# toprakdeviren/gpu-bpe

Hardware: AMD Instinct MI355X
Metric: BPE merges/sec + tokenize GB/s, 1 GiB UTF-8 @ 32K vocab, 1/2/4/8 MI355X (higher is better)
Workload: dtype u16; 1 GPU; headline: 32K-vocab BPE train on 1,073,741,824 B English-like UTF-8 (seed 2, 0.5% 3-byte punctuation), heuristic word boundaries, reference compaction; step = one complete training run (trainer creation + all 32,512 merges) on the HBM-resident corpus; train_bytes=1073741824, target_vocab=32768, parallelism=single

## Files before the change

gpu-bpe_amd/csrc/common.h:

```cpp
#pragma once

#include <hip/hip_runtime.h>
#include <cstdint>
#include <cstdio>
#include <cstdlib>
#include <cstring>
#include <map>
#include <mutex>
#include <string>
#include <type_traits>
#include <unordered_map>
#include <utility>
#include <vector>

#include "../../include/gpubpe.h"

struct GbpePool {
    std::multimap<uint64_t, void*> idle;
    std::unordered_map<void*, uint64_t> busy;
    uint64_t idle_bytes = 0, hits = 0, misses = 0;
};

struct GbpeGrowBuf {
    void* p = nullptr;
// ... 68 lines not shown
        if (p && cap >= n) return hipSuccess;
        GbpeArray nb;
        hipError_t e = nb.reserve(c, n, esz);
        if (e == hipSuccess && p && keep) e = hipMemcpyAsync(nb.p, p, keep * esz, hipMemcpyDeviceToDevice, s);
        if (e == hipSuccess) e = hipStreamSynchronize(s);
        if (e == hipSuccess) *this = std::move(nb);
        return e;
    }
};

int gbpe_set_error(gbpe_ctx* ctx, int code, const char* fmt, ...);

#define GBPE_HIP(ctx, call)                                                              \
    do {                                                                                 \
        hipError_t _e = (call);                                                          \
        if (_e != hipSuccess)                                                            \
            return gbpe_set_error((ctx), _e == hipErrorOutOfMemory ? GBPE_E_OOM           \
                                                                   : GBPE_E_DEVICE,      \
                                  "%s failed: %s (%s:%d)", #call, hipGetErrorString(_e), \
                                  __FILE__, __LINE__);                                   \
    } while (0)

#define GBPE_LAUNCH_CHECK(ctx) GBPE_HIP(ctx, hipGetLastError())

__device__ __forceinline__ uint32_t gbpe_fmix32(uint32_t x) {
    x = (x ^ (x >> 16)) * 0x7feb352du;
    x = (x ^ (x >> 15)) * 0x846ca68bu;
    return x ^ (x >> 16);
}

__host__ __device__ static inline uint64_t gbpe_div_up(uint64_t a, uint64_t b) { return (a + b - 1) / b; }

constexpr const char* kGbpeDebugKeys[] = {
    "lexicon", "lex_check", "rehash", "delta_mt", "zt", "rfl", "rflz", "lxwg", "lxtwo", "pair", "pseg", "prej", "poison",
    "encode_slice", "decode_slice", "dec_plain", "me_cs", "htime", "ptrace", "rtime",
};

inline long gbpe_debug_knob(const char* key, long def) {
    const char* e = getenv("GBPE_DEBUG");
    if (!e) return def;
    const size_t kl = strlen(key);
    for (const char* p = e; *p;) {
        if (!strncmp(p, key, kl) && p[kl] == '=') return strtol(p + kl + 1, nullptr, 10);
        const char* c = strchr(p, ',');
        if (!c) break;
        p = c + 1;
    }
    return def;
}

inline std::string gbpe_debug_unknown() {
    const char* e = getenv("GBPE_DEBUG");
    for (const char* p = e ? e : ""; *p;) {
        const size_t el = strcspn(p, ","), kl = strcspn(p, ",=");
        bool ok = el == 0;
        for (const char* k : kGbpeDebugKeys) ok = ok || (kl < el && strlen(k) == kl && !strncmp(p, k, kl));
        if (!ok) return std::string(p, kl ? kl : el);
        p += el + (p[el] == ',');
    }
    return "";
}

int gbpe_pretok_gpt4_launch(gbpe_ctx* ctx, const uint8_t* d_bytes, uint64_t n, uint8_t* d_ws);
int gbpe_pretok_gpt4_docs_launch(gbpe_ctx* ctx, const uint8_t* d_bytes, uint64_t n, const uint8_t* d_flags, uint8_t* d_ws);
int gbpe_pretok_cl100k_launch(gbpe_ctx* ctx, const uint8_t* d_bytes, uint64_t n, const uint8_t* d_flags, uint8_t* d_ws);
constexpr uint32_t GBPE_DOC_BAD_ORDER = 1u, GBPE_DOC_BAD_FIRST = 2u, GBPE_DOC_BAD_LAST = 4u;
int gbpe_doc_flags_launch(gbpe_ctx* ctx, const uint64_t* d_doc_off, uint64_t n_docs, uint64_t n, uint8_t* d_flags,
// ... 8 lines not shown
```

gpu-bpe_amd/csrc/sparse.h:

```cpp
#pragma once

#include "train_dev.h"

namespace {

constexpr uint32_t SP_WPW_MIN = 16;
constexpr uint32_t SP_CH = 256;
constexpr uint32_t SP_INV = 0xFFFFFFFFu;
constexpr uint32_t SP_SHRINKS = 64;
constexpr uint32_t SP_SHRINKS_MAX = 1024;
constexpr uint32_t SP_SECW = 256;
constexpr uint32_t SP_DIV = 64;
constexpr uint32_t SP_LX_DIV = 16;
constexpr uint32_t SP_SHRINK_PCT = 200;
constexpr uint32_t SP_ZONE_F = 3;
constexpr uint32_t SP_SUB_ZONE = 1u << 20;
constexpr uint32_t SP_SUB_K = 16;
constexpr uint32_t SP_ZSEG_LO = 8192;
constexpr uint32_t SP_BODY_SUB = 4;
constexpr uint32_t SP_BODY_MIN = 256;

constexpr uint32_t SP_SIGW = 64;
__device__ __forceinline__ uint32_t sig_hash(uint32_t pid) { return gbpe_fmix32(pid ^ 0x9E3779B9u); }
__device__ __forceinline__ void sig_bits(uint32_t pid, uint32_t& b1, uint32_t& b2, uint32_t& b3) {
// ... 499 lines not shown
        for (int k = 1; k < ZPT; ++k) xv = k == hk ? x[k] : xv;
        s_last = ((rwm >> hk) & 1u) ? (nw | (xv & WS)) : xv;
    }
    asm volatile("s_waitcnt vmcnt(0)" ::: "memory");
    __syncthreads();
    if (t == 0) {
        constexpr unsigned long long TAG = 1ull << 32;
        __hip_atomic_store(&zg->gran[seg][0], TAG | Ks, __ATOMIC_RELAXED, __HIP_MEMORY_SCOPE_AGENT);
        __hip_atomic_store(&zg->gran[seg][1], TAG | Ts, __ATOMIC_RELAXED, __HIP_MEMORY_SCOPE_AGENT);
        __hip_atomic_store(&zg->gran[seg][2], TAG | (Ks ? (s_last | 0x80000000u) : 0u), __ATOMIC_RELAXED,
                           __HIP_MEMORY_SCOPE_AGENT);
        KT(7);
    }
    constexpr uint32_t PV = 16 / sizeof(S), PVL = sizeof(S) == 2 ? 3 : 2;
    auto swz = [](uint32_t o) -> uint32_t {
        const uint32_t c = o >> PVL;
        return ((c ^ ((c >> 3) & 7u)) << PVL) | (o & (PV - 1u));
    };
    uint32_t wsm = 0;
#pragma unroll
    for (int k = 0; k < ZPT; ++k) {
        const bool rw = (rwm >> k) & 1u;
        const uint32_t v = rw ? (nw | (x[k] & WS)) : x[k];
        wsm |= ((x[k] & WS) ? 1u : 0u) << k;
        const uint32_t o = pre + (uint32_t)__popc(keep & ((1u << k) - 1u));
        S* dst = ((keep >> k) & 1u) ? &xs[swz(o)] : &L.trash[lane];
        *dst = (S)v;
    }
    for (uint32_t r = rwm; r; r &= r - 1) {
        const int k = __ffs(r) - 1;
        zc[gi0 + k] = (S)(nw | (((wsm >> k) & 1u) ? WS : 0u));
    }
    if (wid == 0) {
        uint32_t gk = 0, gt = 0, gl = 0;
        for (uint32_t it = 0;; ++it) {
            bool ok = true;
            if ((uint32_t)lane < nz) {
                const unsigned long long x0 = __hip_atomic_load(&zg->gran[lane][0], __ATOMIC_RELAXED, __HIP_MEMORY_SCOPE_AGENT);
                const unsigned long long x1 = __hip_atomic_load(&zg->gran[lane][1], __ATOMIC_RELAXED, __HIP_MEMORY_SCOPE_AGENT);
                const unsigned long long x2 = __hip_atomic_load(&zg->gran[lane][2], __ATOMIC_RELAXED, __HIP_MEMORY_SCOPE_AGENT);
                ok = (x0 >> 32) == 1u && (x1 >> 32) == 1u && (x2 >> 32) == 1u;
                gk = (uint32_t)x0;
                gt = (uint32_t)x1;
                gl = (uint32_t)x2;
            }
            if (__all(ok)) break;
            if (it > ZSEG_SPIN) {
                if (lane == 0) atomicOr(&st->err, ERR_SPIN);
                break;
            }
            __builtin_amdgcn_s_sleep(1);
        }
        const bool in = (uint32_t)lane < nz;
        uint32_t sp = in && (uint32_t)lane < seg ? gk : 0u, sk = in ? gk : 0u, stt = in ? gt : 0u;
        sp = wave_sum_u32(sp);
        sk = wave_sum_u32(sk);
        stt = wave_sum_u32(stt);
        const unsigned long long hm = __ballot(in && (gl >> 31));
        if (lane == 0) {
            s_pre = sp;
            s_kz = sk;
            s_m = EXACT ? 0u : stt;
            s_x0 = 0u;
        }
        if (hm && lane == 63 - __clzll(hm)) s_x0 = gl & 0x7FFFFFFFu;
    }
    __syncthreads();
    if (t == 0) KT(8);
    const uint32_t P = s_pre, Kz = s_kz, m = s_m;
    for (uint32_t j = t; j < Ks; j += BT) zo[P + j] = xs[swz(j)];
    if (!EXACT && m) {
        const uint32_t w0 = mc - m, f = q0 ? q0 - 1u : 0u;
        const uint32_t lo = q0 > w0 ? q0 : w0;
        for (uint32_t q = lo + t; q < q1; q += BT) {
            const uint32_t x1 = L.wb[q - f];
            const uint32_t x0 = q == w0 ? s_x0 : (uint32_t)L.wb[q - 1u - f];
            zo[Kz + (q - w0)] = (S)x1;
            if (!(x1 & WS) && (x0 & TM) && (x1 & TM)) lds_add(lt, tb, st, ((x0 & TM) << 16) | (x1 & TM), 1u);
        }
    }
    if (t == 0) KT(9);
    lds_flush(lt, tb, st);
    if (t == 0) {
        KT(4);
        if (seg == 0) {
            zst->m = m;
            zst->valid_total = Kz + m + 1u;
        }
        const uint32_t ws = q1 > q0 ? q1 - q0 : 0u;
        atomicAdd(bytes, (uint64_t)sizeof(S) * ((uint64_t)nh + Ks + 2u * ws + (EXACT ? 0u : mc / nz)));
    }
}

struct SelShard {
    uint32_t zf = SP_ZONE_F;
    uint32_t sub = 1;
    uint32_t k2 = 0;
    uint32_t prej = 0;
// ... 1149 lines not shown
```

gpu-bpe_amd/csrc/train.hip:

```cpp


#include <chrono>
#include "trainer.h"

int trainer_create_impl(gbpe_ctx* ctx, const uint8_t* bytes, uint64_t n, const uint8_t* word_starts,
                        int input_on_device, const gbpe_train_opts* opts, uint64_t cap_extra, gbpe_trainer** out,
                        const StateInit* si) {
    if (!ctx || !out || !opts) return gbpe_set_error(ctx, GBPE_E_INVALID, "null argument");
    *out = nullptr;
    if (n == 0) return gbpe_set_error(ctx, GBPE_E_EMPTY, "No symbols to train on — corpus is empty after pre-processing");
    if (!bytes) return gbpe_set_error(ctx, GBPE_E_INVALID, "bytes is null");
    if (n >= 0xFFFFFFF0ull) return gbpe_set_error(ctx, GBPE_E_INVALID, "corpus too large for one device (%llu symbols)", (unsigned long long)n);
    const auto t_create0 = std::chrono::steady_clock::now();
    auto* t = new (std::nothrow) gbpe_trainer();
    if (!t) return gbpe_set_error(ctx, GBPE_E_OOM, "host allocation failed");
    if (const int rc = trainer_config(t, ctx, opts)) {
        delete t;
        return rc;
    }
    const uint32_t next_id = t->next_id0;
    t->bps = t->u16 ? 2 : 4;
    t->n0 = n;
    t->n = (uint32_t)n;
    hipStream_t s = ctx->stream;
// ... 205 lines not shown
            t->ht_filters += std::chrono::duration<double, std::micro>(std::chrono::steady_clock::now() - a0).count();
            ++t->ht_nfilters;
        }
    }
    if (!t->sp && t->h_st->enter_lim && t->n >= (1u << 24)) k = 1;
    if (t->sp && (uint32_t)t->n - t->h_st->B > SP_SUB_ZONE && k > SP_SUB_K) k = SP_SUB_K;
    DevState* hs = t->h_st.p;
    hs->merges_done = 0;
    hs->budget = k;
    if (t->sp) hs->sel_round = 0;
    hipLaunchKernelGGL(k_step_in, dim3(1), dim3(1), 0, s, t->st.p, t->sp ? t->zst.p : (DevState*)nullptr, k);
#ifdef GBPE_KTRACE
    if (getenv("GBPE_KTRACE_OUT")) {
        static unsigned long long* kbuf = nullptr;
        if (!kbuf) {
            const size_t nb = (size_t)(KT_MERGES / KT_EVERY) * 2 * KT_WG * KT_SLOTS * 8;
            TR_HIP(t, dev_malloc(t->ctx, &kbuf, nb));
            TR_HIP(t, hipMemsetAsync(kbuf, 0, nb, s));
            TR_HIP(t, hipMemcpyToSymbolAsync(HIP_SYMBOL(g_ktr), &kbuf, sizeof(kbuf), 0, hipMemcpyHostToDevice, s));
        }
        const uint32_t kb = (uint32_t)t->done;
        TR_HIP(t, hipMemcpyToSymbolAsync(HIP_SYMBOL(g_kt_base), &kb, 4, 0, hipMemcpyHostToDevice, s));
    }
#endif
    const uint64_t ntiles = gbpe_div_up(t->n, TILE);
    const uint32_t g_tail = (t->flags & GBPE_TRAIN_EXACT_COMPACTION) ? 0u
                            : grid_persistent(t->ctx, gbpe_div_up(t->n / 2 + 1, TPB * 16), 1);
    const uint32_t g_delta = (uint32_t)(ntiles ? ntiles : 1);
    const uint32_t g_compact = (uint32_t)ntiles + g_tail;
    uint32_t g_refresh = t->g_refresh;
    const bool timing = (t->flags & GBPE_TRAIN_TIMING) != 0;
    const bool sparse = t->sp;
    SpGrid sg{};
    if (sparse) {
        const uint32_t zn = (uint32_t)t->n - hs->B;
        const uint64_t zt = gbpe_div_up(zn, TILE);
        const uint32_t z256 = t->u16 ? zone_max<uint16_t>(256) : zone_max<uint32_t>(256);
        sg.bt = zn <= z256 ? 256 : 1024;
        body_grid(t, sg.bt, &sg.body, &sg.wpg, 0, &sg.sub);
        if (sg.bt == 1024 && t->u16 && zn <= 16384u) sg.bt = 1023;
        sg.zone1 = zn <= (t->u16 ? zone_max<uint16_t>(sg.bt) : zone_max<uint32_t>(sg.bt)) ? 1u : 0u;
        const bool p16 = t->pair_on && t->pair16_on && t->zseg.p && k >= 2 && zn > SP_ZSEG_LO && zn <= SP_PAIR16_HI;
        if (p16) {
            sg.bt = 1022;
            sg.zone1 = 1;
        } else if (t->zseg.p && zn > SP_ZSEG_LO && zn <= NSEG_MAX * 16384u) {
            sg.seg8 = zn <= NSEG_MAX * 8192u;
            sg.zone1 = (uint32_t)gbpe_div_up(zn, sg.seg8 ? 8192u : 16384u);
        }
        sg.copy = (t->flags & GBPE_TRAIN_EXACT_COMPACTION) ? 0u : grid_persistent(t->ctx, gbpe_div_up(zn / 5 + 1, TPB * 8), 1);
        sg.zdelta = (uint32_t)(zt ? zt : 1);
        sg.zcompact = (uint32_t)zt + ((t->flags & GBPE_TRAIN_EXACT_COMPACTION) ? 0u
                                      : grid_persistent(t->ctx, gbpe_div_up(zn / 2 + 1, TPB * 16), 1));
        const uint32_t extra = p16 ? ((t->flags & GBPE_TRAIN_EXACT_COMPACTION) ? 1u : 2u) : sg.zone1 ? sg.zone1 : sg.copy;
        if (sg.bt >= 1022 && extra && sg.body + extra > t->body_cap && 2 * extra <= t->body_cap)
            body_grid(t, sg.bt, &sg.body, &sg.wpg, t->body_cap - extra, &sg.sub);
        if (t->refresh_late && zn <= t->refresh_late_z) {
            const uint32_t want = std::min<uint32_t>(t->tb.nblk,
                                                     std::max<uint32_t>(t->refresh_late, (uint32_t)gbpe_div_up(t->tb.nblk, TPB)));
            if (want != t->g_refresh) {
                t->g_refresh = g_refresh = want;
                if (t->u16)
                    GBPE_LAUNCH_REFRESH(uint16_t, want, t->tb.nblk, s, t->st.p, 0u, 0, t->tb, (uint16_t*)nullptr,
                                        (const uint32_t*)nullptr, (DevState*)nullptr, (uint32_t*)nullptr, FusedSel(),
                                        t->part.p, (uint32_t*)nullptr);
                else
                    GBPE_LAUNCH_REFRESH(uint32_t, want, t->tb.nblk, s, t->st.p, 0u, 0, t->tb, (uint32_t*)nullptr,
                                        (const uint32_t*)nullptr, (DevState*)nullptr, (uint32_t*)nullptr, FusedSel(),
                                        t->part.p, (uint32_t*)nullptr);
                GBPE_LAUNCH_CHECK(t->ctx);
            }
        }
        sg.refresh = g_refresh;
        sg.pair = t->pair_on && sg.zone1 == 1 && (sg.bt == 256 || sg.bt == 1022) && t->zseg.p && k >= 2;
    }
    uint32_t nl = k;
    if (sg.pair) nl = std::min<uint32_t>(k, (uint32_t)std::ceil((double)k / (1.0 + t->pair_rate)) + 2u);
    const uint32_t paired0 = hs->paired;
    auto launch_all = [&]() -> int {
        for (uint32_t r = 0; r < nl; ++r) {
            hipEvent_t* ev = timing ? &t->evs[5 * r] : nullptr;
            int rc;
            if (sparse)
                rc = t->u16 ? launch_merge_sparse<uint16_t>(t, r, s, sg, timing, ev)
                            : launch_merge_sparse<uint32_t>(t, r, s, sg, timing, ev);
            else
                rc = t->u16 ? launch_merge<uint16_t>(t, r, s, g_delta, g_compact, g_refresh, timing, ev)
                            : launch_merge<uint32_t>(t, r, s, g_delta, g_compact, g_refresh, timing, ev);
            if (rc != GBPE_OK) return rc;
        }
        return GBPE_OK;
    };
    const auto h0 = std::chrono::steady_clock::now();
    auto h1 = h0;
    {
        int rc = launch_all();
        if (rc != GBPE_OK) return rc;
        h1 = std::chrono::steady_clock::now();
        const bool cl = sparse && t->d_clog.p;
        hipLaunchKernelGGL(k_step_out, dim3(1), dim3(1024), 0, s, t->st.p, sparse ? t->zst.p : (DevState*)nullptr, t->tb,
                           sparse ? 1 : 0, (const uint32_t*)t->d_log.p, k * 4u, (const uint32_t*)(cl ? t->d_clog.p : nullptr),
                           cl ? k * 2u : 0u, t->h_st.p, t->h_zst.p, t->h_log.p, cl ? t->h_clog.p : (uint32_t*)nullptr);
        GBPE_LAUNCH_CHECK(t->ctx);
    }
    TR_HIP(t, hipStreamSynchronize(s));
    const uint32_t done = hs->merges_done;
    {
        const uint32_t dbl = hs->paired - paired0;
        t->pair_done += dbl;
        if (sg.pair && done > dbl) t->pair_rate = (double)dbl / (double)(done - dbl);
        if (t->ptrace)
            fprintf(stderr, "[ptrace] merge %u zone %u zone1 %u bt %d pair %d launches %u done %u paired %u cand %u mc %u us %.1f\n",
                    t->done, hs->n - hs->B, sg.zone1, sg.bt, sg.pair ? 1 : 0, nl, done, dbl,
                    hs->pair_cand, done ? t->h_log.p[(done - 1) * 4 + 3] : 0u,
                    std::chrono::duration<double, std::micro>(std::chrono::steady_clock::now() - hs0).count());
    }
    if (t->htime) {
        t->ht_pre += std::chrono::duration<double, std::micro>(h0 - hs0).count();
        const double enq = std::chrono::duration<double, std::micro>(h1 - h0).count();
        const double wait = std::chrono::duration<double, std::micro>(std::chrono::steady_clock::now() - h1).count();
        t->ht_enq += enq;
        t->ht_wait += wait;
        ++t->ht_steps;
        if (sparse && (uint32_t)t->n - hs->B <= 16384u) {
            t->ht_enq_late += enq;
            t->ht_wait_late += wait;
            ++t->ht_steps_late;
            t->ht_merges_late += done;
        }
    }
#ifdef GBPE_BSPROF
    if (sparse && getenv("GBPE_BSPROF")) {
        unsigned long long h[8] = {0, 0, 0, 0, 0, 0, 0, 0};
        TR_HIP(t, hipMemcpyFromSymbol(h, HIP_SYMBOL(g_bsprof), sizeof(h), 0, hipMemcpyDeviceToHost));
        fprintf(stderr, "[bsprof] merges %u-%u waves %llu sectors %llu passes %llu | cyc/sector loads+hits %.0f deltas %.0f "
                        "writes %.0f flush %.0f | sector-phase cyc/wave %.0f\n",
                (unsigned)t->done, (unsigned)(t->done + done), h[7], h[5], h[4], h[5] ? (double)h[0] / h[5] : 0.0,
                h[5] ? (double)h[1] / h[5] : 0.0, h[5] ? (double)h[2] / h[5] : 0.0, h[5] ? (double)h[3] / h[5] : 0.0,
                h[7] ? (double)h[6] / h[7] : 0.0);
        const unsigned long long z[8] = {0, 0, 0, 0, 0, 0, 0, 0};
        TR_HIP(t, hipMemcpyToSymbol(HIP_SYMBOL(g_bsprof), z, sizeof(z), 0, hipMemcpyHostToDevice));
    }
#endif
    const uint32_t err = hs->err | (sparse ? t->h_zst->err : 0u);
    if (err) {
        return gbpe_set_error(t->ctx, GBPE_E_INTERNAL, "training invariant violated (err=0x%x: %s%s%s%s%s)", err,
                              (err & ERR_TABLE_FULL) ? "pair table full " : "",
                              (err & ERR_COUNT_MISMATCH) ? "survivor count mismatch " : "",
// ... 334 lines not shown
```

gpu-bpe_amd/csrc/train_dev.h:

```cpp
#pragma once

#include "common.h"
#include "scan.h"

#include <algorithm>
#include <chrono>
#include <type_traits>
#include <cstdarg>

namespace {

constexpr int TPB = 256;
constexpr int EPT = 32;
constexpr int TILE = TPB * EPT;
constexpr int LTAB = 2048;
constexpr int LTAB_FULL = 8192;
constexpr int LPROBE = 24;
constexpr uint32_t BLK_LOG2 = 8;
constexpr int SEL_THREADS = 1024;

template <typename S> struct Sym;
template <> struct Sym<uint16_t> { static constexpr uint32_t WS = 0x8000u, TM = 0x7FFFu; };
template <> struct Sym<uint32_t> { static constexpr uint32_t WS = 0x10000u, TM = 0xFFFFu; };

// ... 67 lines not shown
    uint32_t ndirty;
    uint32_t err;
    uint32_t valid_total;
    uint32_t budget;
    uint32_t live;
    uint64_t tail_total;
    uint32_t max_live;
    uint32_t epoch;
    uint32_t B;
    uint32_t Bp;
    uint32_t body_rm;
    uint32_t sp_abort;
    uint32_t sel_round;
    uint64_t sp_bytes;
    uint32_t zlast;
    uint32_t is_last;
    uint32_t cand;
    uint32_t hitsec;
    uint32_t mc_prev;
    uint32_t enter_lim;
    uint32_t mc2;
    uint32_t body_rm2;
    uint32_t acc2;
    uint32_t paired;
    uint32_t pair_cand;
    uint32_t pair_rej;
};
static_assert(sizeof(DevState) <= 256, "state");

__device__ __forceinline__ uint64_t win_src0(const DevState& g, uint32_t mc) {
    return (uint64_t)(uint32_t)(g.n - g.Bp) - 2ull * mc;
}

constexpr uint32_t NSEG_MAX = 64;
constexpr uint32_t ZSEG_SPIN = 1u << 22;
struct ZSegState {
    uint32_t ticket;
    uint32_t pad[15];
    unsigned long long gran[NSEG_MAX][4];
};
constexpr uint32_t ZSEG_WORDS = 16 + NSEG_MAX * 8;

#ifdef GBPE_KTRACE
constexpr uint32_t KT_MERGES = 40000, KT_EVERY = 16, KT_WG = 2048, KT_SLOTS = 12;
__constant__ unsigned long long* g_ktr;
__constant__ uint32_t g_kt_base;
__device__ __forceinline__ void kt_put(uint32_t round, uint32_t wg, int i, unsigned long long v) {
    const uint32_t m = g_kt_base + round;
    if (g_ktr && m < KT_MERGES && m % KT_EVERY == 0 && wg < 2 * KT_WG)
        g_ktr[((uint64_t)(m / KT_EVERY) * 2 * KT_WG + wg) * KT_SLOTS + i] = v;
}
#define KT(i) kt_put(round, blockIdx.x, (i), wall_clock64())
#define KTV(i, v) kt_put(round, blockIdx.x, (i), (v))
#define KTR(i) kt_put(round, KT_WG + blockIdx.x, (i), wall_clock64())
#define KTW(i) do { if ((threadIdx.x & 63) == 0 && threadIdx.x < 256) kt_put(round, KT_WG - 8u + (threadIdx.x >> 6), (i), wall_clock64()); } while (0)
#define KTC(i) do { if ((threadIdx.x & 63) == 0 && threadIdx.x < 256) kt_put(round, KT_WG - 4u + (threadIdx.x >> 6), (i), wall_clock64()); } while (0)
#else
#define KTW(i) ((void)0)
#define KTC(i) ((void)0)
#define KT(i) ((void)0)
#define KTV(i, v) ((void)0)
#define KTR(i) ((void)0)
#endif

#ifdef GBPE_BSPROF
__device__ unsigned long long g_bsprof[8];
#define BSP_ARG , unsigned long long (&bsp)[6]
#define BSP_PASS , bsp
#define BSP_CLK(v) const unsigned long long v = clock64()
#define BSP_ADD(i, x) bsp[i] += (x)
#else
#define BSP_ARG
#define BSP_PASS
#define BSP_CLK(v) ((void)0)
// ... 441 lines not shown
            if (i0 + k < n && i0 + k > 0 && !(x & Sym<S>::WS) && t0 && t1 && (t0 >> 7) == half)
                atomicAdd(&hist[((t0 & 127u) << 8) | t1], 1u);
            prev = x;
        }
    }
    __syncthreads();
    for (int i = threadIdx.x; i < 32768; i += CB_T) {
        const uint32_t c = hist[i];
        if (c) atomicAdd(&gh[(half << 15) | (uint32_t)i], c);
    }
}

__device__ void table_add(const Table& tb, DevState* st, uint32_t pid, uint32_t delta);
__global__ __launch_bounds__(256) void k_count_hist(const uint32_t* __restrict__ gh, DevState* st, Table tb) {
    const uint32_t i = blockIdx.x * 256u + threadIdx.x;
    const uint32_t c = gh[i];
    if (c) table_add(tb, st, ((i >> 8) << 16) | (i & 255u), c);
}

__device__ void select_merge(DevState* st, Table tb, uint32_t* __restrict__ log, uint32_t* __restrict__ grpsum,
                             DevState* zst, uint32_t exact);

struct FusedSel {
    uint32_t* log = nullptr;
    uint32_t* grpsum = nullptr;
    uint32_t exact = 0;
};


template <typename S, bool WIDE = false>
__global__ __launch_bounds__(TPB) void k_refresh(DevState* st, uint32_t round, int finish, Table tb, S* __restrict__ cur,
                                                 const uint32_t* __restrict__ rwlist, DevState* zst,
                                                 uint32_t* __restrict__ clog = nullptr, FusedSel fs = FusedSel(),
                                                 uint64_t* __restrict__ part = nullptr, uint32_t* __restrict__ zseg = nullptr) {
    (void)cur;
    if (zseg && blockIdx.x == 0)
        for (uint32_t i = threadIdx.x; i < ZSEG_WORDS; i += TPB)
            if (i == 0 || i >= 16) zseg[i] = 0u;
    (void)rwlist;
    if (part && finish == 2 && threadIdx.x == 0) KTR(0);
    __shared__ uint64_t s_dmask[WIDE ? TPB / 64 : 1];
    __shared__ uint64_t s_bm[WIDE ? TPB : 64], s_bm2[WIDE ? TPB : 64];
    const uint32_t per = (tb.nblk + gridDim.x - 1) / gridDim.x;
    constexpr bool wide = WIDE;
    const uint32_t b0 = blockIdx.x * per;
    uint64_t f_bm = 0ull, f_bm2 = 0ull;
    bool f_d = false;
    if (wide || threadIdx.x < 64) {
        const uint32_t blk = b0 + threadIdx.x;
        const bool in = threadIdx.x < per && blk < tb.nblk;
        if (part && in) {
            f_bm = tb.bmax[blk];
            f_bm2 = tb.bmax2[blk];
        }
        f_d = in && tb.dirty[blk];
    }
    if (finish && blockIdx.x == 0) {
        constexpr int NW = sizeof(DevState) / 4;
        __shared__ union {
            DevState d;
            uint32_t w[NW];
        } s_g, s_z;
        static_assert(64 + 2 * NW <= TPB, "state snapshot beside the flag loads");
        if (threadIdx.x >= 64 && threadIdx.x < 64 + NW)
            s_g.w[threadIdx.x - 64] = reinterpret_cast<const uint32_t*>(st)[threadIdx.x - 64];
        else if (zst && threadIdx.x >= 64 + NW && threadIdx.x < 64 + 2 * NW)
            s_z.w[threadIdx.x - 64 - NW] = reinterpret_cast<const uint32_t*>(zst)[threadIdx.x - 64 - NW];
        __syncthreads();
        const DevState& g = s_g.d;
        const DevState& z = s_z.d;
        const uint32_t r = finish >= 2 ? g.merges_done : round;
// ... 996 lines not shown
```

gpu-bpe_amd/csrc/trainer.h:

```cpp
#pragma once

#include <cmath>

#include "train_dev.h"
#include <chrono>
#include "sparse.h"




struct gbpe_trainer {
    gbpe_ctx* ctx = nullptr;
    bool u16 = true;
    uint32_t bps = 2;
    uint64_t n0 = 0, cap_syms = 0;
    uint64_t n_prev0 = 0;
    uint32_t next_id0 = 256;
    GbpeArray<void> buf[2];
    int cur = 0;
    uint64_t n = 0;
    uint32_t needed = 0, done = 0;
    bool stop = false;
    uint32_t flags = 0, batch = GBPE_BATCH_SIZE;
    GbpeArray<DevState> st;
// ... 30 lines not shown
    int zcur = 0;
    GbpeArray<DevState> zst;
    GbpeArray<DevState, true> h_zst;
    GbpeArray<uint32_t> d_u32;
    GbpeArray<uint64_t> part;
    GbpeArray<uint2> zdr_out;
    GbpeArray<uint32_t> zdr_offs, zdr_flag;
    uint32_t zdr_ntile = 0;
    GbpeArray<uint32_t> zseg;
    uint32_t table_grows = 0;
    GbpeArray<uint64_t> wg_bytes;
    uint32_t delta_mt = 2048;
    double ms_sparse = 0, ms_dense = 0;
    double ms_body = 0;
    double ms_create = 0;
    uint64_t dense_bytes = 0;
    uint32_t g_refresh = 0;
    uint64_t sp_merges = 0, sp_sectors = 0, sp_zone = 0;
    uint32_t sp_enters = 0, sp_exits = 0;
    uint32_t sp_cooldown = 0;
    GbpeArray<uint32_t> d_bhist;
    uint32_t lx_wg = 16384;
    bool lx_two = true;
    uint32_t lx_resize = 0;
    uint32_t sp_zt = 5;
    uint32_t refresh_late = 64;
    uint32_t refresh_late_z = 16384;
    bool rehash_on = true;
    uint32_t body_cap = 256;
    bool pair_on = true;
    double pair_rate = 0.5;
    uint64_t pair_done = 0;
    bool pair16_on = true;
    uint32_t pair_prej = 0;
    uint32_t ptrace = 0;
    GbpeArray<uint32_t> d_clog;
    GbpeArray<uint32_t, true> h_clog;
    FILE* trace = nullptr;
    uint32_t htime = 0;
    double ht_enq = 0, ht_wait = 0, ht_enq_late = 0, ht_wait_late = 0, ht_pre = 0, ht_post = 0, ht_out = 0;
    double ht_shrink = 0, ht_filters = 0, ht_grow = 0;
    uint64_t ht_nshrink = 0, ht_nfilters = 0;
    std::chrono::steady_clock::time_point ht_last{};
    uint64_t ht_steps = 0, ht_steps_late = 0, ht_merges_late = 0;
    bool lex = false;
    bool lex_on = true;
    bool lex_only = false;
    GbpeArray<void> lx_store;
    GbpeArray<uint32_t> lx_mul;
    uint64_t lx_len = 0;
    GbpeArray<uint32_t> lx_occ;
    uint64_t lx_nocc = 0;
    GbpeArray<uint32_t> lx_w0;
    uint32_t lx_nuid = 0;
    GbpeArray<void> lx_tmp;
    uint64_t lx_words = 0, lx_builds = 0, lx_fallbacks = 0;
};

namespace {

int tr_err(gbpe_trainer* t, int code, const char* msg) { return gbpe_set_error(t->ctx, code, "%s", msg); }

#define TR_HIP(t, call) GBPE_HIP((t)->ctx, call)

inline void* sp_body(const gbpe_trainer* t) { return t->lex ? t->lx_store.p : t->buf[t->bcur].p; }
inline uint32_t* sp_mul(const gbpe_trainer* t) { return t->lex ? t->lx_mul.p : nullptr; }
// ... 136 lines not shown
                               t->hitmask.p, t->tile_cnt.p, t->grpsum.p, g_delta, 0xFFFFFFFFu);
        if (timing) TR_HIP(t, hipEventRecord(ev[3], s));
        hipLaunchKernelGGL((k_compact<S, true>), dim3(g_compact), dim3(CTPB), 0, s, t->st.p, round, cur, oth,
                           (const uint32_t*)t->hitmask.p, (const uint32_t*)t->tile_cnt.p, (const uint32_t*)t->grpsum.p, t->tb);
    } else {
        if (mt)
            hipLaunchKernelGGL((k_delta_mt<S, false, 8>), dim3(g_mt + g_mtail), dim3(TPB), 0, s, t->st.p, round,
                               (const S*)cur, t->tb, t->hitmask.p, t->tile_cnt.p, t->grpsum.p, g_delta, g_mt, 0u, ZdrView());
        else
            hipLaunchKernelGGL((k_delta<S, false>), dim3(g_delta + g_dtail), dim3(TPB), 0, s, t->st.p, round, (const S*)cur,
                               t->tb, t->hitmask.p, t->tile_cnt.p, t->grpsum.p, g_delta, g_delta);
        if (timing) TR_HIP(t, hipEventRecord(ev[3], s));
        hipLaunchKernelGGL((k_compact<S, false>), dim3(g_compact), dim3(CTPB), 0, s, t->st.p, round, cur, oth,
                           (const uint32_t*)t->hitmask.p, (const uint32_t*)t->tile_cnt.p, (const uint32_t*)t->grpsum.p, t->tb);
    }
    if (timing) TR_HIP(t, hipEventRecord(ev[2], s));
    FusedSel fs;
    fs.log = nullptr;
    fs.grpsum = t->grpsum.p;
    fs.exact = exact ? 1u : 0u;
    GBPE_LAUNCH_REFRESH(S, g_refresh, t->tb.nblk, s, t->st.p, round, 1, t->tb, cur, (const uint32_t*)nullptr,
                        (DevState*)nullptr, (uint32_t*)nullptr, fs, (uint64_t*)nullptr, (uint32_t*)nullptr);
    if (timing) TR_HIP(t, hipEventRecord(ev[4], s));
    GBPE_LAUNCH_CHECK(t->ctx);
    return GBPE_OK;
}


struct SpGrid {
    uint32_t body, copy, zdelta, zcompact, refresh;
    uint32_t wpg = 16;
    uint32_t sub = 1;
    bool seg8 = false;
    uint32_t zone1;
    int bt;
    bool pair = false;
};

constexpr uint32_t SP_PAIR16_HI = 16384;

template <typename S>
uint32_t zone_max(int bt) {
    return bt == 1023 ? 1024u * 16u : bt == 1022 ? SP_PAIR16_HI : bt == 1024 ? ZoneDim<S, 1024>::ZMAX : ZoneDim<S, 256>::ZMAX;
}
inline void body_grid(const gbpe_trainer* t, int bt, uint32_t* nbody, uint32_t* wpg, uint32_t cap = 0,
                      uint32_t* sub = nullptr) {
    const uint32_t W = (uint32_t)gbpe_div_up(t->nsec, 32);
    const uint32_t minw = bt == 1024 ? 32u : 16u;
    uint32_t g = (uint32_t)gbpe_div_up(W, minw);
    const uint32_t gmin = std::min<uint32_t>(W, SP_BODY_MIN);
    if (g < gmin) g = gmin;
    if (g > (cap ? cap : t->body_cap)) g = cap ? cap : t->body_cap;
    if (g == 0) g = 1;
    *wpg = (uint32_t)gbpe_div_up(W, g);
    if (*wpg == 0) *wpg = 1;
    *nbody = (uint32_t)gbpe_div_up(W, *wpg);
    if (*nbody == 0) *nbody = 1;
    if (sub) {
        *sub = 1;
        const uint32_t c = cap ? cap : t->body_cap;
        while (*sub * 2 <= SP_BODY_SUB && (uint64_t)W * *sub * 2 <= c) *sub *= 2;
        if (*sub > 1) {
            *wpg = 1;
            *nbody = W * *sub;
        }
    }
}

template <typename S, bool EXACT, typename... A>
void launch_body(int bt, uint32_t grid, hipStream_t s, A... args) {
    if (bt == 1022)
        hipLaunchKernelGGL((k_body<S, EXACT, 512, 32, false, true>), dim3(grid), dim3(512), 0, s, args...);
    else if (bt == 2048)
        hipLaunchKernelGGL((k_body<S, EXACT, 1024, 16, true>), dim3(grid), dim3(1024), 0, s, args...);
    else if (bt == 2049)
        hipLaunchKernelGGL((k_body<S, EXACT, 1024, 8, true>), dim3(grid), dim3(1024), 0, s, args...);
    else if (bt == 1023 && sizeof(S) == 2)
        hipLaunchKernelGGL((k_body<S, EXACT, 1024, 16>), dim3(grid), dim3(1024), 0, s, args...);
    else if (bt >= 1023)
        hipLaunchKernelGGL((k_body<S, EXACT, 1024>), dim3(grid), dim3(1024), 0, s, args...);
    else
        hipLaunchKernelGGL((k_body<S, EXACT, 256>), dim3(grid), dim3(256), 0, s, args...);
}

template <typename S>
int launch_merge_sparse(gbpe_trainer* t, uint32_t round, hipStream_t s, const SpGrid& g, bool timing, hipEvent_t* ev) {
    S* zc = (S*)t->zbuf[t->zcur ^ (round & 1)].p;
    S* zo = (S*)t->zbuf[t->zcur ^ (round & 1) ^ 1].p;
    const bool exact = (t->flags & GBPE_TRAIN_EXACT_COMPACTION) != 0;
    if (timing) TR_HIP(t, hipEventRecord(ev[0], s));
    if (timing) TR_HIP(t, hipEventRecord(ev[1], s));
    const bool inbody = g.zone1 >= 2;
    const uint32_t z1 = g.zone1;
    const int bt = inbody ? (g.seg8 ? 2049 : 2048) : g.bt;
    SelShard sh;
    sh.sub = g.sub;
    sh.k2 = g.pair ? 1u : 0u;
    sh.prej = t->pair_prej;
    sh.churn = (g.pair && !exact && (bt == 256 || bt == 1022) && z1 == 1) ? 1u : 0u;
    const uint32_t gb = g.body + (g.zone1 ? g.zone1 : g.copy) + sh.churn;
    if ((uint64_t)g.body + 1 > t->wg_bytes.cap)
        return gbpe_set_error(t->ctx, GBPE_E_INTERNAL, "k_body grid (%u) above its byte counters (%llu)", g.body,
                              (unsigned long long)t->wg_bytes.cap);
    S* zb0 = (S*)t->zbuf[t->zcur].p;
    S* zb1 = (S*)t->zbuf[t->zcur ^ 1].p;
    if (exact)
        launch_body<S, true>(bt, gb, s, t->st.p, round, (S*)sp_body(t), t->sec.p, t->bits.p, t->W, g.wpg, t->sig.p, t->tb,
                             g.body, zb1, (S*)t->wtmp.p, t->d_clog.p ? 1u : 0u, t->zst.p, zb0, z1,
                             (const uint64_t*)t->part.p, g.refresh, t->d_log.p, t->grpsum.p, t->wg_bytes.p, t->tb, sh,
                             sp_mul(t), (ZSegState*)t->zseg.p);
    else
        launch_body<S, false>(bt, gb, s, t->st.p, round, (S*)sp_body(t), t->sec.p, t->bits.p, t->W, g.wpg, t->sig.p, t->tb,
                              g.body, zb1, (S*)t->wtmp.p, t->d_clog.p ? 1u : 0u, t->zst.p, zb0, z1,
                              (const uint64_t*)t->part.p, g.refresh, t->d_log.p, t->grpsum.p, t->wg_bytes.p, t->tb, sh,
                              sp_mul(t), (ZSegState*)t->zseg.p);
    if (timing) TR_HIP(t, hipEventRecord(ev[3], s));
    if (!g.zone1 && !exact) {
        const bool mt = t->delta_mt && g.zdelta >= t->delta_mt;
        const uint32_t g_mt = (uint32_t)gbpe_div_up(g.zdelta, 8);
        const uint32_t ntw = mt ? g_mt : g.zdelta;
        const uint32_t gch = (uint32_t)std::min<uint64_t>(ZDR_P, std::max<uint64_t>(1, gbpe_div_up(((uint32_t)t->n - t->h_st->B) / 5 + 1, 16384)));
        ZdrView zv;
        zv.out = t->zdr_out.p;
        zv.offs = t->zdr_offs.p;
        zv.flag = t->zdr_flag.p;
        zv.ntile = ntw;
        zv.tag = (uint32_t)(t->done + round + 1);
        if (ntw > t->zdr_ntile) return gbpe_set_error(t->ctx, GBPE_E_INTERNAL, "zone delta dumps too small");
        if (mt)
            hipLaunchKernelGGL((k_delta_mt<S, false, 8>), dim3(g_mt), dim3(TPB), 0, s, t->zst.p, round, (const S*)zc, t->tb,
                               t->hitmask.p, t->tile_cnt.p, t->grpsum.p, g.zdelta, g_mt, 0u, zv);
        else
            hipLaunchKernelGGL((k_delta<S, false, true>), dim3(g.zdelta), dim3(TPB), 0, s, t->zst.p, round, (const S*)zc,
                               t->tb, t->hitmask.p, t->tile_cnt.p, t->grpsum.p, g.zdelta, g.zdelta, zv);
        hipLaunchKernelGGL((k_compact<S, false, true>), dim3(g.zdelta), dim3(CTPB), 0, s, t->zst.p, round, zc, zo,
                           (const uint32_t*)t->hitmask.p, (const uint32_t*)t->tile_cnt.p, (const uint32_t*)t->grpsum.p, t->tb,
                           (const S*)t->wtmp.p, (const DevState*)t->st.p, 1u);
        hipLaunchKernelGGL(k_churn<S>, dim3(gch), dim3(CH_BT), 0, s, t->zst.p, round, zc, zo, (const uint32_t*)t->hitmask.p,
                           (const uint32_t*)t->grpsum.p, (const S*)t->wtmp.p, t->tb, zv, ntw);
        hipLaunchKernelGGL(k_zdr, dim3(ZDR_P), dim3(TPB), 0, s, zv, ntw + gch, t->tb, t->zst.p, round);
    } else if (!g.zone1) {
        const uint32_t g_mt = (uint32_t)gbpe_div_up(g.zdelta, 8);
        if (t->delta_mt && g.zdelta >= t->delta_mt)
            hipLaunchKernelGGL((k_delta_mt<S, true, 8>), dim3(g_mt), dim3(TPB), 0, s, t->zst.p, round, (const S*)zc, t->tb,
                               t->hitmask.p, t->tile_cnt.p, t->grpsum.p, g.zdelta, g_mt);
        else
            hipLaunchKernelGGL((k_delta<S, true, true>), dim3(g.zdelta), dim3(TPB), 0, s, t->zst.p, round, (const S*)zc,
                               t->tb, t->hitmask.p, t->tile_cnt.p, t->grpsum.p, g.zdelta, 0xFFFFFFFFu);
        hipLaunchKernelGGL((k_compact<S, true, true>), dim3(g.zcompact), dim3(CTPB), 0, s, t->zst.p, round, zc, zo,
                           (const uint32_t*)t->hitmask.p, (const uint32_t*)t->tile_cnt.p, (const uint32_t*)t->grpsum.p,
                           t->tb, (const S*)t->wtmp.p, (const DevState*)t->st.p);
    }
    if (timing) TR_HIP(t, hipEventRecord(ev[2], s));
    GBPE_LAUNCH_REFRESH(S, g.refresh, t->tb.nblk, s, t->st.p, round, 2, t->tb, (S*)nullptr, (const uint32_t*)nullptr,
                        t->zst.p, t->d_clog.p, FusedSel(), t->part.p, t->zseg.p);
    if (timing) TR_HIP(t, hipEventRecord(ev[4], s));
    GBPE_LAUNCH_CHECK(t->ctx);
    return GBPE_OK;
}

__global__ void k_restride(const uint32_t* __restrict__ old, uint32_t w_old, uint32_t* __restrict__ nb, uint32_t w_new,
                           uint64_t rows) {
    const uint64_t tot = rows * w_new;
    for (uint64_t i = (uint64_t)blockIdx.x * blockDim.x + threadIdx.x; i < tot; i += (uint64_t)gridDim.x * blockDim.x) {
        const uint64_t r = i / w_new, w = i % w_new;
        nb[i] = w < w_old ? old[r * w_old + w] : 0u;
    }
}

int sp_scratch(gbpe_trainer* t, uint64_t cap) {
    TR_HIP(t, t->sp_loc.reserve(t->ctx, cap));
    TR_HIP(t, t->sp_blk.reserve(t->ctx, gbpe_div_up(cap, SCAN_BLK) + 1));
    return GBPE_OK;
}

int sp_wg_bytes(gbpe_trainer* t, uint64_t W) {
    hipStream_t s = t->ctx->stream;
    const uint64_t need = std::max<uint64_t>(gbpe_div_up(W, SP_WPW_MIN), t->body_cap) + 2, had = t->wg_bytes.cap;
    if (need <= had) return GBPE_OK;
    TR_HIP(t, t->wg_bytes.reserve_keep(t->ctx, need, had, s));
    TR_HIP(t, hipMemsetAsync(t->wg_bytes.p + had, 0, (need - had) * sizeof(uint64_t), s));
    return GBPE_OK;
}

int sp_reserve(gbpe_trainer* t, uint64_t need_sec, uint64_t need_store, uint64_t need_occ) {
    hipStream_t s = t->ctx->stream;
    if (need_sec > t->sec.cap || need_sec > (uint64_t)t->W * 32 || need_sec * SP_SIGW > t->sig.cap ||
        need_sec > t->sp_loc.cap || (t->lex && need_sec > t->lx_w0.cap)) {
// ... 608 lines not shown
    uint64_t sl = t->zbuf[0].cap;
    if (Bp + sl > t->cap_syms) sl = t->cap_syms - Bp;
    TR_HIP(t, hipMemcpyAsync(body + Bp, t->zbuf[t->zcur ^ 1].p, sl * t->bps, hipMemcpyDeviceToDevice, s));
    hs->sp_abort = 0;
    TR_HIP(t, hipMemcpyAsync(&t->st->sp_abort, &hs->sp_abort, 4, hipMemcpyHostToDevice, s));
    TR_HIP(t, hipStreamSynchronize(s));
    if (btot != B) return gbpe_set_error(t->ctx, GBPE_E_INTERNAL, "sparse exit: body sectors hold %llu symbols, expected %u",
                                         (unsigned long long)btot, B);
    t->cur = t->bcur ^ 1;
    t->sp = false;
    t->lex = false;
    ++t->sp_exits;
    return GBPE_OK;
}

int trainer_config(gbpe_trainer* t, gbpe_ctx* ctx, const gbpe_train_opts* opts) {
    const std::string bad = gbpe_debug_unknown();
    if (!bad.empty()) return gbpe_set_error(ctx, GBPE_E_INVALID, "GBPE_DEBUG: unknown key '%s'", bad.c_str());
    t->ctx = ctx;
    t->flags = opts->flags;
    t->batch = opts->batch_size ? opts->batch_size : GBPE_BATCH_SIZE;
    const uint32_t vocab_size = opts->vocab_size ? opts->vocab_size : 256u;
    const uint32_t next_id = opts->next_token_id ? opts->next_token_id : 256u;
    t->next_id0 = next_id;
    t->needed = opts->target_vocab_size > vocab_size ? opts->target_vocab_size - vocab_size : 0u;
    const uint64_t max_id = (uint64_t)next_id + t->needed;
    t->u16 = max_id <= 0x8000ull;
    t->max_id = (uint32_t)(max_id < 0x10000ull ? max_id : 0x10000ull);
    t->body_cap = (uint32_t)(ctx->num_cu > 0 ? ctx->num_cu : 256);
    t->lex_on = gbpe_debug_knob("lexicon", 1) != 0;
    t->pair_on = gbpe_debug_knob("pair", 1) != 0;
    t->pair16_on = gbpe_debug_knob("pseg", 1) != 0;
    t->pair_prej = (uint32_t)std::max<long>(0, gbpe_debug_knob("prej", 0));
    t->ptrace = (uint32_t)gbpe_debug_knob("ptrace", 0);
    t->rehash_on = gbpe_debug_knob("rehash", 1) != 0;
    t->delta_mt = (uint32_t)gbpe_debug_knob("delta_mt", t->delta_mt);
    t->sp_zt = (uint32_t)gbpe_debug_knob("zt", t->sp_zt);
    t->refresh_late = (uint32_t)gbpe_debug_knob("rfl", t->refresh_late);
    t->refresh_late_z = (uint32_t)gbpe_debug_knob("rflz", t->refresh_late_z);
    t->lx_wg = (uint32_t)std::max<long>(1, gbpe_debug_knob("lxwg", t->lx_wg));
    t->lx_two = gbpe_debug_knob("lxtwo", 1) != 0;
    t->htime = (uint32_t)gbpe_debug_knob("htime", 0);
    if (t->sp_zt < SP_ZONE_F) t->sp_zt = SP_ZONE_F;
    if (const char* e = getenv("GBPE_SPARSE_TRACE")) {
        t->trace = fopen(e, "w");
        if (t->trace && (t->d_clog.reserve(ctx, (size_t)t->batch * 2) != hipSuccess ||
                         t->h_clog.reserve(ctx, (size_t)t->batch * 2) != hipSuccess))
            t->d_clog.release(), t->h_clog.release();
    }
    t->bps = t->u16 ? 2 : 4;
    return GBPE_OK;
}

int sp_exit_any(gbpe_trainer* t) { return !t->sp ? GBPE_OK : (t->u16 ? sp_exit<uint16_t>(t) : sp_exit<uint32_t>(t)); }

}

struct StateInit {
    const uint32_t* prev;
    uint64_t n_prev;
};
int trainer_create_impl(gbpe_ctx* ctx, const uint8_t* bytes, uint64_t n, const uint8_t* word_starts,
                        int input_on_device, const gbpe_train_opts* opts, uint64_t cap_extra, gbpe_trainer** out,
                        const StateInit* si = nullptr);
```

Before: 64790 merges/s.

## Extend segmented zone body to 128 segments and add 32K-segment u16 variant

Raises the segmented-zone cap from 64 to 128 segments, limited by CU count, and adds a seg32 path that uses 32768-element segments for u16 symbols. The in-kernel cross-segment scan now handles two granules per lane when there are more than 64 segments. The refresh kernel clears only as many zseg words as are in use. The aim is to keep larger zones on the single-launch segmented body path instead of falling back to the slower non-segmented path. The cost is a more complex spin-wait over more granules and heavier per-thread work in the seg32 body.

Measured after the change: 66390 merges/s (median of 6 runs). +2.5%, better.

```diff
diff --git a/gpu-bpe_amd/csrc/common.h b/gpu-bpe_amd/csrc/common.h
--- a/gpu-bpe_amd/csrc/common.h
+++ b/gpu-bpe_amd/csrc/common.h
@@ -124,7 +124,7 @@
 __host__ __device__ static inline uint64_t gbpe_div_up(uint64_t a, uint64_t b) { return (a + b - 1) / b; }
 
 constexpr const char* kGbpeDebugKeys[] = {
-    "lexicon", "lex_check", "rehash", "delta_mt", "zt", "rfl", "rflz", "lxwg", "lxtwo", "pair", "pseg", "prej", "poison",
+    "lexicon", "lex_check", "rehash", "delta_mt", "zt", "rfl", "rflz", "lxwg", "lxtwo", "pair", "pseg", "prej", "zsmax", "zs32", "poison",
     "encode_slice", "decode_slice", "dec_plain", "me_cs", "htime", "ptrace", "rtime",
 };
 
diff --git a/gpu-bpe_amd/csrc/sparse.h b/gpu-bpe_amd/csrc/sparse.h
--- a/gpu-bpe_amd/csrc/sparse.h
+++ b/gpu-bpe_amd/csrc/sparse.h
@@ -555,38 +555,66 @@
         zc[gi0 + k] = (S)(nw | (((wsm >> k) & 1u) ? WS : 0u));
     }
     if (wid == 0) {
-        uint32_t gk = 0, gt = 0, gl = 0;
-        for (uint32_t it = 0;; ++it) {
-            bool ok = true;
-            if ((uint32_t)lane < nz) {
-                const unsigned long long x0 = __hip_atomic_load(&zg->gran[lane][0], __ATOMIC_RELAXED, __HIP_MEMORY_SCOPE_AGENT);
-                const unsigned long long x1 = __hip_atomic_load(&zg->gran[lane][1], __ATOMIC_RELAXED, __HIP_MEMORY_SCOPE_AGENT);
-                const unsigned long long x2 = __hip_atomic_load(&zg->gran[lane][2], __ATOMIC_RELAXED, __HIP_MEMORY_SCOPE_AGENT);
-                ok = (x0 >> 32) == 1u && (x1 >> 32) == 1u && (x2 >> 32) == 1u;
-                gk = (uint32_t)x0;
-                gt = (uint32_t)x1;
-                gl = (uint32_t)x2;
-            }
-            if (__all(ok)) break;
-            if (it > ZSEG_SPIN) {
-                if (lane == 0) atomicOr(&st->err, ERR_SPIN);
-                break;
-            }
-            __builtin_amdgcn_s_sleep(1);
-        }
-        const bool in = (uint32_t)lane < nz;
+        const uint32_t sh = (uint32_t)lane + 64u;
+        const bool in = (uint32_t)lane < nz, inh = sh < nz;
+        const bool up = nz > 64u;
+        uint32_t gk = 0, gt = 0, gl = 0, hk = 0, ht = 0, hl = 0;
+        auto sweep = [&](auto two) {
+            constexpr bool TWO = decltype(two)::value;
+            for (uint32_t it = 0;; ++it) {
+                bool ok = true;
+                if (in) {
+                    const unsigned long long x0 = __hip_atomic_load(&zg->gran[lane][0], __ATOMIC_RELAXED, __HIP_MEMORY_SCOPE_AGENT);
+                    const unsigned long long x1 = __hip_atomic_load(&zg->gran[lane][1], __ATOMIC_RELAXED, __HIP_MEMORY_SCOPE_AGENT);
+                    const unsigned long long x2 = __hip_atomic_load(&zg->gran[lane][2], __ATOMIC_RELAXED, __HIP_MEMORY_SCOPE_AGENT);
+                    ok = (x0 >> 32) == 1u && (x1 >> 32) == 1u && (x2 >> 32) == 1u;
+                    gk = (uint32_t)x0;
+                    gt = (uint32_t)x1;
+                    gl = (uint32_t)x2;
+                    if constexpr (TWO) {
+                        if (inh) {
+                            const unsigned long long y0 = __hip_atomic_load(&zg->gran[sh][0], __ATOMIC_RELAXED, __HIP_MEMORY_SCOPE_AGENT);
+                            const unsigned long long y1 = __hip_atomic_load(&zg->gran[sh][1], __ATOMIC_RELAXED, __HIP_MEMORY_SCOPE_AGENT);
+                            const unsigned long long y2 = __hip_atomic_load(&zg->gran[sh][2], __ATOMIC_RELAXED, __HIP_MEMORY_SCOPE_AGENT);
+                            ok = ok && (y0 >> 32) == 1u && (y1 >> 32) == 1u && (y2 >> 32) == 1u;
+                            hk = (uint32_t)y0;
+                            ht = (uint32_t)y1;
+                            hl = (uint32_t)y2;
+                        }
+                    }
+                }
+                if (__all(ok)) break;
+                if (it > ZSEG_SPIN) {
+                    if (lane == 0) atomicOr(&st->err, ERR_SPIN);
+                    break;
+                }
+                __builtin_amdgcn_s_sleep(1);
+            }
+        };
+        if (up) sweep(std::true_type());
+        else sweep(std::false_type());
         uint32_t sp = in && (uint32_t)lane < seg ? gk : 0u, sk = in ? gk : 0u, stt = in ? gt : 0u;
+        if (up) {
+            sp += inh && sh < seg ? hk : 0u;
+            sk += inh ? hk : 0u;
+            stt += inh ? ht : 0u;
+        }
         sp = wave_sum_u32(sp);
         sk = wave_sum_u32(sk);
         stt = wave_sum_u32(stt);
         const unsigned long long hm = __ballot(in && (gl >> 31));
+        const unsigned long long hmh = up ? __ballot(inh && (hl >> 31)) : 0ull;
         if (lane == 0) {
             s_pre = sp;
             s_kz = sk;
             s_m = EXACT ? 0u : stt;
             s_x0 = 0u;
         }
-        if (hm && lane == 63 - __clzll(hm)) s_x0 = gl & 0x7FFFFFFFu;
+        if (hmh) {
+            if (lane == 63 - __clzll(hmh)) s_x0 = hl & 0x7FFFFFFFu;
+        } else if (hm && lane == 63 - __clzll(hm)) {
+            s_x0 = gl & 0x7FFFFFFFu;
+        }
     }
     __syncthreads();
     if (t == 0) KT(8);
diff --git a/gpu-bpe_amd/csrc/train.hip b/gpu-bpe_amd/csrc/train.hip
--- a/gpu-bpe_amd/csrc/train.hip
+++ b/gpu-bpe_amd/csrc/train.hip
@@ -261,6 +261,7 @@
     const bool timing = (t->flags & GBPE_TRAIN_TIMING) != 0;
     const bool sparse = t->sp;
     SpGrid sg{};
+    const uint32_t zn0 = sparse ? (uint32_t)t->n - hs->B : 0u;
     if (sparse) {
         const uint32_t zn = (uint32_t)t->n - hs->B;
         const uint64_t zt = gbpe_div_up(zn, TILE);
@@ -273,9 +274,13 @@
         if (p16) {
             sg.bt = 1022;
             sg.zone1 = 1;
-        } else if (t->zseg.p && zn > SP_ZSEG_LO && zn <= NSEG_MAX * 16384u) {
-            sg.seg8 = zn <= NSEG_MAX * 8192u;
+        } else if (t->zseg.p && zn > SP_ZSEG_LO && zn <= t->zseg_max * 16384u &&
+                   !(t->u16 && t->zseg32 == 2 && zn > 64u * 16384u)) {
+            sg.seg8 = zn <= std::min<uint32_t>(t->zseg_max, 64u) * 8192u;
             sg.zone1 = (uint32_t)gbpe_div_up(zn, sg.seg8 ? 8192u : 16384u);
+        } else if (t->zseg.p && t->u16 && t->zseg32 && zn > SP_ZSEG_LO && zn <= t->zseg_max * 32768u) {
+            sg.seg32 = true;
+            sg.zone1 = (uint32_t)gbpe_div_up(zn, 32768u);
         }
         sg.copy = (t->flags & GBPE_TRAIN_EXACT_COMPACTION) ? 0u : grid_persistent(t->ctx, gbpe_div_up(zn / 5 + 1, TPB * 8), 1);
         sg.zdelta = (uint32_t)(zt ? zt : 1);
@@ -339,10 +344,10 @@
         t->pair_done += dbl;
         if (sg.pair && done > dbl) t->pair_rate = (double)dbl / (double)(done - dbl);
         if (t->ptrace)
-            fprintf(stderr, "[ptrace] merge %u zone %u zone1 %u bt %d pair %d launches %u done %u paired %u cand %u mc %u us %.1f\n",
-                    t->done, hs->n - hs->B, sg.zone1, sg.bt, sg.pair ? 1 : 0, nl, done, dbl,
+            fprintf(stderr, "[ptrace] merge %u zone %u zone1 %u bt %d pair %d launches %u done %u paired %u cand %u mc %u us %.1f zone0 %u\n",
+                    t->done, hs->n - hs->B, sg.zone1, sg.seg32 ? 2050 : sg.bt, sg.pair ? 1 : 0, nl, done, dbl,
                     hs->pair_cand, done ? t->h_log.p[(done - 1) * 4 + 3] : 0u,
-                    std::chrono::duration<double, std::micro>(std::chrono::steady_clock::now() - hs0).count());
+                    std::chrono::duration<double, std::micro>(std::chrono::steady_clock::now() - hs0).count(), zn0);
     }
     if (t->htime) {
         t->ht_pre += std::chrono::duration<double, std::micro>(h0 - hs0).count();
diff --git a/gpu-bpe_amd/csrc/train_dev.h b/gpu-bpe_amd/csrc/train_dev.h
--- a/gpu-bpe_amd/csrc/train_dev.h
+++ b/gpu-bpe_amd/csrc/train_dev.h
@@ -123,14 +123,14 @@
     return (uint64_t)(uint32_t)(g.n - g.Bp) - 2ull * mc;
 }
 
-constexpr uint32_t NSEG_MAX = 64;
+constexpr uint32_t NSEG_MAX = 128;
 constexpr uint32_t ZSEG_SPIN = 1u << 22;
 struct ZSegState {
     uint32_t ticket;
     uint32_t pad[15];
     unsigned long long gran[NSEG_MAX][4];
 };
-constexpr uint32_t ZSEG_WORDS = 16 + NSEG_MAX * 8;
+__host__ __device__ constexpr uint32_t zseg_words(uint32_t nz) { return nz >= 2 ? 16u + (nz < NSEG_MAX ? nz : NSEG_MAX) * 8u : 1u; }
 
 #ifdef GBPE_KTRACE
 constexpr uint32_t KT_MERGES = 40000, KT_EVERY = 16, KT_WG = 2048, KT_SLOTS = 12;
@@ -638,11 +638,17 @@
 __global__ __launch_bounds__(TPB) void k_refresh(DevState* st, uint32_t round, int finish, Table tb, S* __restrict__ cur,
                                                  const uint32_t* __restrict__ rwlist, DevState* zst,
                                                  uint32_t* __restrict__ clog = nullptr, FusedSel fs = FusedSel(),
-                                                 uint64_t* __restrict__ part = nullptr, uint32_t* __restrict__ zseg = nullptr) {
+                                                 uint64_t* __restrict__ part = nullptr, uint32_t* __restrict__ zseg = nullptr,
+                                                 uint32_t zseg_nz = 0) {
     (void)cur;
-    if (zseg && blockIdx.x == 0)
-        for (uint32_t i = threadIdx.x; i < ZSEG_WORDS; i += TPB)
-            if (i == 0 || i >= 16) zseg[i] = 0u;
+    const uint32_t nwz = zseg_words(zseg_nz);
+    if (zseg && blockIdx.x == 0) {
+#pragma unroll
+        for (uint32_t r = 0; r < (zseg_words(NSEG_MAX) + TPB - 1) / TPB; ++r) {
+            const uint32_t i = threadIdx.x + r * TPB;
+            if (i < nwz && (i == 0 || i >= 16)) zseg[i] = 0u;
+        }
+    }
     (void)rwlist;
     if (part && finish == 2 && threadIdx.x == 0) KTR(0);
     __shared__ uint64_t s_dmask[WIDE ? TPB / 64 : 1];
diff --git a/gpu-bpe_amd/csrc/trainer.h b/gpu-bpe_amd/csrc/trainer.h
--- a/gpu-bpe_amd/csrc/trainer.h
+++ b/gpu-bpe_amd/csrc/trainer.h
@@ -86,6 +86,8 @@
     double pair_rate = 0.5;
     uint64_t pair_done = 0;
     bool pair16_on = true;
+    uint32_t zseg_max = NSEG_MAX;
+    uint32_t zseg32 = 1;
     uint32_t pair_prej = 0;
     uint32_t ptrace = 0;
     GbpeArray<uint32_t> d_clog;
@@ -288,12 +290,19 @@
     uint32_t wpg = 16;
     uint32_t sub = 1;
     bool seg8 = false;
+    bool seg32 = false;
     uint32_t zone1;
     int bt;
     bool pair = false;
 };
 
 constexpr uint32_t SP_PAIR16_HI = 16384;
+
+inline uint32_t zseg_cap(uint32_t num_cu, long want) {
+    const uint32_t room = std::max<uint32_t>(64u, num_cu / 2);
+    const uint32_t w = (uint32_t)std::min<long>(std::max<long>(want, 2), (long)NSEG_MAX);
+    return std::min(w, room);
+}
 
 template <typename S>
 uint32_t zone_max(int bt) {
@@ -331,6 +340,10 @@
         hipLaunchKernelGGL((k_body<S, EXACT, 1024, 16, true>), dim3(grid), dim3(1024), 0, s, args...);
     else if (bt == 2049)
         hipLaunchKernelGGL((k_body<S, EXACT, 1024, 8, true>), dim3(grid), dim3(1024), 0, s, args...);
+    else if (bt == 2050) {
+        if constexpr (sizeof(S) == 2)
+            hipLaunchKernelGGL((k_body<S, EXACT, 1024, 32, true>), dim3(grid), dim3(1024), 0, s, args...);
+    }
     else if (bt == 1023 && sizeof(S) == 2)
         hipLaunchKernelGGL((k_body<S, EXACT, 1024, 16>), dim3(grid), dim3(1024), 0, s, args...);
     else if (bt >= 1023)
@@ -348,7 +361,7 @@
     if (timing) TR_HIP(t, hipEventRecord(ev[1], s));
     const bool inbody = g.zone1 >= 2;
     const uint32_t z1 = g.zone1;
-    const int bt = inbody ? (g.seg8 ? 2049 : 2048) : g.bt;
+    const int bt = inbody ? (g.seg32 ? 2050 : g.seg8 ? 2049 : 2048) : g.bt;
     SelShard sh;
     sh.sub = g.sub;
     sh.k2 = g.pair ? 1u : 0u;
@@ -409,7 +422,7 @@
     }
     if (timing) TR_HIP(t, hipEventRecord(ev[2], s));
     GBPE_LAUNCH_REFRESH(S, g.refresh, t->tb.nblk, s, t->st.p, round, 2, t->tb, (S*)nullptr, (const uint32_t*)nullptr,
-                        t->zst.p, t->d_clog.p, FusedSel(), t->part.p, t->zseg.p);
+                        t->zst.p, t->d_clog.p, FusedSel(), t->part.p, t->zseg.p, inbody ? z1 : 0u);
     if (timing) TR_HIP(t, hipEventRecord(ev[4], s));
     GBPE_LAUNCH_CHECK(t->ctx);
     return GBPE_OK;
@@ -1084,6 +1097,8 @@
     t->pair_on = gbpe_debug_knob("pair", 1) != 0;
     t->pair16_on = gbpe_debug_knob("pseg", 1) != 0;
     t->pair_prej = (uint32_t)std::max<long>(0, gbpe_debug_knob("prej", 0));
+    t->zseg_max = zseg_cap(t->body_cap, gbpe_debug_knob("zsmax", NSEG_MAX));
+    t->zseg32 = (uint32_t)gbpe_debug_knob("zs32", t->zseg32);
     t->ptrace = (uint32_t)gbpe_debug_knob("ptrace", 0);
     t->rehash_on = gbpe_debug_knob("rehash", 1) != 0;
     t->delta_mt = (uint32_t)gbpe_debug_knob("delta_mt", t->delta_mt);
```
